# DreamWaterFound/self_commit_ORB-SLAM2

Measured on AMD Instinct MI355X. Metric: frames/s ORB extract+match (1000 feat, 640x480), higher is better.
Workload: dtype u8; 1 GPU; batch of 256 synthetic 640x480 frames per GPU (8 distinct resident batches per step, one launch set per batch), ORB extract (1000 feat, 8 levels, FAST 20/7) + brute-force Hamming SearchByBoW of consecutive frames; batch_per_gpu=256, streams=3, width=640, height=480, nfeatures=1000, parallelism=frames sharded, 1 rank(s), no data-path collective

## Files before the change

### self_commit_orb-slam2_amd/csrc/orbx_extractor.hip

```cpp
#include <math.h>
#include <stdarg.h>
#include <stdio.h>
#include <stdlib.h>
#include <string.h>

#include <algorithm>
#include <atomic>
#include <chrono>
#include <condition_variable>
#include <functional>
#include <memory>
#include <mutex>
#include <thread>
#include <vector>

#include "orbx_internal.h"

static thread_local char g_err[512] = "";

void orbx_set_error(const char *fmt, ...)
{
    va_list ap;
    va_start(ap, fmt);
    vsnprintf(g_err, sizeof(g_err), fmt, ap);
// ... 40 lines not shown
    OrbxGeom geom;
    bool geomValid = false;
    std::vector<uint8_t> binHost;
    std::vector<uint32_t> rsHost;
    std::vector<OrbxFcCell> fcHost;
    OrbxDevBuf<OrbxPyrTile> ptDev;
    int ptBatchW = 0, ptBatchH = 0;
    int ptTiles = 0, ptLds = 0, ptTab = 0;
    int nodeCap = 512;
    hipStream_t stream = nullptr;
    hipEvent_t ev[ORBX_PROF_RING][ST_COUNT + 1] = {};
    bool profiling = false;
    int profCount = 0;
    bool debugTaps = false;
    DevBuf<OrbxGeom> geomDev;
    DevBuf<uint8_t> binDev, pyr, blur, score, staging;
    DevBuf<uint32_t> rsDev;
    DevBuf<OrbxFcCell> fcDev;
    DevBuf<int> cellCount, lvlCnt, lvlBase, status;
    DevBuf<uint8_t> outArena[2];
    int *outCntP[2] = {nullptr, nullptr};
    int *outStP[2] = {nullptr, nullptr};
    orbx_keypoint *outKpP[2] = {nullptr, nullptr};
    uint8_t *outDescP[2] = {nullptr, nullptr};
    size_t arenaKpOff = 0, arenaDescOff = 0, arenaBytes = 0;
    hipEvent_t consumerEv[2] = {nullptr, nullptr};
    hipEvent_t pyrConsumerEv = nullptr;
    int cur = 0;
    DevBuf<uint32_t> cellSlots, ptBuf, labBuf;
    DevBuf<OrbxLevelKp> lvlKp;
    int allocBatch = 0;
    int lastBatch = 0;
    bool lastPyrFast = false;
    bool lastChunked = false;
    const uint8_t *lastImg0 = nullptr;
    int lastStride = 0;
    size_t lastFramePitch = 0;
    uint8_t *hostStaging = nullptr;
    size_t hostStagingBytes = 0;
    int stagingStride = 0;
    size_t stagingFramePitch = 0;
    uint8_t *hostOut = nullptr;
    size_t hostOutBytes = 0;
    hipGraph_t sgGraph[2] = {nullptr, nullptr};
    hipGraphExec_t sgExec[2] = {nullptr, nullptr};
    bool sgValid = false;
    bool sgDisabled = false;
    struct Combiner *comb = nullptr;
    bool combDisabled = false;
    orbx_extractor *expectPartner = nullptr;
    bool isEngine = false;
    size_t hostPyrOff = 0;
    bool hostPyrValid = false;
    bool hostSynced = false;
    bool lastCombined = false;
    struct PipeSlot {
        uint8_t *hostIn = nullptr; size_t hostInBytes = 0;
        DevBuf<uint8_t> devIn;
        uint8_t *hostRes = nullptr; size_t hostResBytes = 0;
        const uint8_t **ptrTab = nullptr; size_t ptrTabBytes = 0;
        hipEvent_t evUp = nullptr, evKern = nullptr, evDown = nullptr;
        int batch = 0, cap = 0;
        size_t offKp = 0, offDesc = 0, offSt = 0;
    } pipe[2];
    int pipeHead = 0, pipeCount = 0;
    double pipeUs[4] = {0, 0, 0, 0};
// ... 195 lines not shown
            if (((ln.w + 3) >> 2) * ((dy - (int)h->rsHost[(size_t)lv.bandOff + b] + 7) >> 3) > ORBX_BAND_MAX_ITEMS) {
                orbx_set_error("level %d (%dx%d): a pyramid band resizes more than %d work items of level %d", l, lv.w, lv.h, ORBX_BAND_MAX_ITEMS, l + 1);
                return ORBX_ERR_ARG;
            }
        }
        h->rsHost.push_back((uint32_t)ln.h);
    }
    h->rsHost.insert(h->rsHost.end(), 16, 0u);
    if (maxWCell > 64 || maxHCell > 63) { orbx_set_error("cell %dx%d larger than the detector supports", maxWCell, maxHCell); return ORBX_ERR_ARG; }
    g.fcPitch = maxWCell <= 32 ? 48 : maxWCell <= 48 ? 64 : 80;
    g.fcScPitch = maxWCell <= 42 ? 48 : 80;
    {
        int maxAw = 1;
        for (int l = 0; l < nl; l++) {
            const OrbxLevel &lv = g.lv[l];
            const int maxBX = lv.w - ORBX_BORDER;
            for (int cj = 0; cj < lv.nCols; cj++) {
                const int iniX = ORBX_BORDER + cj * lv.wCell, maxX = std::min(iniX + lv.wCell + 6, maxBX);
                maxAw = std::max(maxAw, (maxX - 3) - (iniX + 3));
            }
        }
        g.fcScPitch = maxAw + 2 <= 48 ? 48 : 80;
        if (g.fcScPitch == 80) g.fcPitch = 80;
    }
    { const char *pe = getenv("ORBX_FC_PITCH"); if (pe && atoi(pe) == 80 && g.fcPitch == 64) g.fcPitch = 80; }
    {
        const int units = (maxHCell + 6) * ((maxWCell + 6 + 15) / 16), ns = (units + 63) / 64;
        g.fcNS = ns <= 2 ? 2 : ns <= 3 ? 3 : ns <= 4 ? 4 : 6;
    }
    g.fcInBytes = g.fcPitch * (maxHCell + 6);
    g.fcScBytes = g.fcScPitch * (maxHCell + 2);
    g.fcLdsBytes = g.fcInBytes + g.fcScBytes + (int)align_up((size_t)maxWCell * maxHCell * 2, 16);
    g.pyrFast = g.pyrBand && (size_t)ORBX_PF_WAVES * (size_t)g.fcLdsBytes <= 48 * 1024 ? 1 : 0;
    h->fcHost.assign((size_t)cells, OrbxFcCell{});
    for (int l = 0; l < nl; l++) {
        const OrbxLevel &lv = g.lv[l];
        const int maxBX = lv.w - ORBX_BORDER, maxBY = lv.h - ORBX_BORDER;
        for (int ci = 0; ci < lv.nRows; ci++)
            for (int cj = 0; cj < lv.nCols; cj++) {
                const int cell = ci * lv.nCols + cj;
                OrbxFcCell &e = h->fcHost[(size_t)lv.cellBase + cell];
                const int iniX = ORBX_BORDER + cj * lv.wCell, iniY = ORBX_BORDER + ci * lv.hCell;
                const int maxX = std::min(iniX + lv.wCell + 6, maxBX), maxY = std::min(iniY + lv.hCell + 6, maxBY);
                const int x0 = iniX + 3, x1 = maxX - 3, y0 = iniY + 3, y1 = maxY - 3, aw = x1 - x0, ah = y1 - y0;
                const bool valid = !(iniY >= maxBY - 3 || iniX >= maxBX - 6 || aw <= 0 || ah <= 0);
                e.xy = valid ? ((uint32_t)x0 | ((uint32_t)y0 << 16)) : ((uint32_t)ORBX_EDGE | ((uint32_t)ORBX_EDGE << 16));
                const int ew = valid ? aw : 1, eh = valid ? ah : 1, nu = (ew + 6 + 15) / 16;
                e.dim = (uint32_t)ew | ((uint32_t)eh << 8) | ((uint32_t)l << 16) | (valid ? 1u << 24 : 0u);
                e.inv = (uint32_t)((65536 + nu - 1) / nu); e.units = (uint32_t)nu | ((uint32_t)((eh + 6) * nu) << 8);
                e.pitch = lv.pitch; e.off = (uint32_t)lv.off;
                e.slot = (uint32_t)(lv.slotBase + cell * lv.cellCap); e.cap = (uint32_t)lv.cellCap;
            }
    }
    g.pyrBytes = align_up(off + 256, 256);
    if (maxNodes > 2048) { orbx_set_error("per-level feature quota %d exceeds the quadtree node capacity 2048", maxNodes); return ORBX_ERR_ARG; }
    h->nodeCap = maxNodes <= 256 ? 256 : (maxNodes <= 512 ? 512 : (maxNodes <= 1024 ? 1024 : 2048));
    const long long keyLimit = 1ll << (32 - (h->nodeCap == 256 ? 8 : h->nodeCap == 512 ? 9 : h->nodeCap == 1024 ? 10 : 11));
    for (int l = 0; l < nl; l++)
        if ((long long)g.lv[l].nCols * g.lv[l].nRows * g.lv[l].cellCap >= keyLimit) {
            orbx_set_error("level %d (%dx%d) can hold %lld FAST candidates, the quadtree's sort key %lld at %d nodes per level", l, g.lv[l].w, g.lv[l].h,
                           (long long)g.lv[l].nCols * g.lv[l].nRows * g.lv[l].cellCap, keyLimit - 1, h->nodeCap);
            return ORBX_ERR_ARG;
        }
    return ORBX_OK;
}

// ... 82 lines not shown
    int rc = ensure_geometry(h, W, H, batch);
    if (rc != ORBX_OK) return rc;
    OrbxLaunch L;
    h->cur ^= 1;
    const int cb = h->cur;
    fill_launch(h, L, img0Dev, batch, stride, framePitch, cb);
    const bool prof = h->profiling;
    hipEvent_t *ev = h->ev[h->profCount % ORBX_PROF_RING];
    if (h->pyrConsumerEv) { ORBX_HIP_CHECK(hipStreamWaitEvent(h->stream, h->pyrConsumerEv, 0)); h->pyrConsumerEv = nullptr; }
    ORBX_HIP_CHECK(hipMemsetAsync(h->status.p, 0, (size_t)(batch + 1) * sizeof(int), h->stream));
    if (prof) ORBX_HIP_CHECK(hipEventRecord(ev[0], h->stream));
    static const bool batchTiles = getenv("ORBX_BATCH_PYR_TILES") && getenv("ORBX_BATCH_PYR_TILES")[0] == '1';
    bool tiled = false;
    if (batchTiles && h->allocBatch > 1) {
        if (h->ptBatchW != W || h->ptBatchH != H) {
            std::vector<OrbxPyrTile> plan;
            h->ptTiles = 0;
            if (plan_pyramid_tiles(h, plan, h->ptTiles, h->ptLds, h->ptTab)) {
                if ((rc = h->ptDev.ensure(plan.size())) != ORBX_OK) return rc;
                ORBX_HIP_CHECK(hipMemcpy(h->ptDev.p, plan.data(), plan.size() * sizeof(OrbxPyrTile), hipMemcpyHostToDevice));
            } else h->ptTiles = 0;
            h->ptBatchW = W; h->ptBatchH = H;
        }
        if (h->ptTiles > 0) {
            L.pyrTiles = h->ptDev.p; L.pyrTileCount = h->ptTiles; L.pyrTileBuf = h->ptLds; L.pyrTileTab = h->ptTab;
            if ((rc = orbx_launch_pyramid_tiles(L)) != ORBX_OK) return rc;
            tiled = true;
        }
    }
    const char *es = getenv("ORBX_PYR_SPLIT");
    L.pyrBand = !tiled && h->geom.pyrBand && !(es && es[0] == '1');
    const char *ef = getenv("ORBX_FAST_SPLIT");
    const bool pyrFast = L.pyrBand && orbx_pyr_fast_applies(L) && !(ef && ef[0] == '1');
    const int nJoin = pyrFast ? std::min(ORBX_PF_JOIN_LEVELS, h->geom.nlevels) : 0;
    if (L.pyrBand) {
        for (int l = 0; l < h->geom.nlevels; l++)
            if ((rc = l < nJoin ? orbx_launch_pyr_band_fast(L, l) : orbx_launch_pyr_band(L, l)) != ORBX_OK) return rc;
    } else if (!tiled)
        for (int l = 1; l < h->geom.nlevels; l++)
            if ((rc = orbx_launch_resize(L, l)) != ORBX_OK) return rc;
    if (prof) ORBX_HIP_CHECK(hipEventRecord(ev[ST_PYR + 1], h->stream));
    L.fcCellFirst = nJoin < h->geom.nlevels ? h->geom.lv[nJoin].cellBase : h->geom.cellsPerFrame;
    if (L.fcCellFirst < h->geom.cellsPerFrame && (rc = orbx_launch_fast_cells(L)) != ORBX_OK) return rc;
    if (prof) ORBX_HIP_CHECK(hipEventRecord(ev[ST_FAST + 1], h->stream));
    if ((rc = orbx_launch_octree(L)) != ORBX_OK) return rc;
    if (prof) ORBX_HIP_CHECK(hipEventRecord(ev[ST_OCTREE + 1], h->stream));
    if (prof) ORBX_HIP_CHECK(hipEventRecord(ev[ST_ORIENT + 1], h->stream));
    if (!L.pyrBand && (rc = orbx_launch_blur(L)) != ORBX_OK) return rc;
    if (prof) ORBX_HIP_CHECK(hipEventRecord(ev[ST_BLUR + 1], h->stream));
    if (h->consumerEv[cb]) { ORBX_HIP_CHECK(hipStreamWaitEvent(h->stream, h->consumerEv[cb], 0)); h->consumerEv[cb] = nullptr; }
    if ((rc = orbx_launch_orient_describe(L)) != ORBX_OK) return rc;
    if (prof) { ORBX_HIP_CHECK(hipEventRecord(ev[ST_DESC + 1], h->stream)); h->profCount++; }
    h->lastBatch = batch; h->lastImg0 = img0Dev; h->lastStride = stride; h->lastFramePitch = framePitch;
    h->lastCombined = false; h->hostSynced = false; h->lastChunked = false; h->lastPyrFast = pyrFast;
    return ORBX_OK;
}

extern "C" int orbx_debug_last_batch_pyr_fast(orbx_extractor *h) { return h && h->lastPyrFast ? 1 : 0; }

static int host_copy_threads()
{
    static const int n = [] {
        const char *e = getenv("ORBX_HOST_COPY_THREADS");
        int v = e && *e ? atoi(e) : (int)std::min(16u, std::max(1u, std::thread::hardware_concurrency() / 2));
        return v < 1 ? 1 : v > 64 ? 64 : v;
    }();
    return n;
}
struct CopyPool {
    std::mutex m;
    std::mutex jm;
    std::condition_variable cvWork, cvDone;
    std::vector<std::thread> workers;
    std::function<void(int, int)> job;
    int n = 0, parts = 0, gen = 0, pending = 0;
    bool stop = false;
    void worker(int id)
    {
        int seen = 0;
        for (;;) {
            std::function<void(int, int)> fn;
            int n_, parts_;
            {
                std::unique_lock<std::mutex> lk(jm);
                cvWork.wait(lk, [&] { return stop || gen != seen; });
                if (stop) return;
                seen = gen; fn = job; n_ = n; parts_ = parts;
            }
            if (id < parts_) fn((int)((long long)n_ * id / parts_), (int)((long long)n_ * (id + 1) / parts_));
            {
                std::lock_guard<std::mutex> lk(jm);
// ... 1504 lines not shown
```

### self_commit_orb-slam2_amd/csrc/orbx_internal.h

```cpp
#ifndef ORBX_INTERNAL_H
#define ORBX_INTERNAL_H

#include <hip/hip_runtime.h>
#include <cstring>
#include <stdint.h>

#include "../../include/orbx.h"

#define ORBX_MAX_LEVELS 12
#define ORBX_EDGE 19
#define ORBX_BORDER 16
#define ORBX_HALF_PATCH 15
#define ORBX_PATCH 31
#define ORBX_CELL_W 30
#define ORBX_MAX_INI 8

#define ORBX_DEV_ERR_PTCAP 1
#define ORBX_DEV_ERR_NODECAP 2
#define ORBX_DEV_ERR_KPCAP 4

struct OrbxLevel {
    int w, h, pitch;
    int off;
    int nCols, nRows, wCell, hCell;
// ... 10 lines not shown
    int bandOff;
    uint32_t bandDivNc, bandDivG4;
    double rsScaleX, rsScaleY;
    int rsColOff, rsRowOff;
    int patchSize;
    float scale;
};

struct OrbxGeom {
    int nlevels, W, H;
    int iniTh, minTh;
    int cellsPerFrame, slotsPerFrame, kpPerFrame, outCap;
    int blurTiles;
    int fcPitch, fcScPitch, fcNS;
    int fcInBytes, fcScBytes, fcLdsBytes;
    size_t pyrBytes;
    int pyrBand;
    int pyrFast;
    uint32_t taps[7];
    int umax[16];
    OrbxLevel lv[ORBX_MAX_LEVELS];
};

#define ORBX_BAND_MAX_ITEMS (1 << 14)
static inline uint32_t orbx_band_div(int n)
{
    uint32_t S = 14;
    while ((1u << (S - 14)) < (uint32_t)n) S++;
    const uint32_t m = (uint32_t)((((uint64_t)1 << S) + (uint64_t)n - 1) / (uint64_t)n);
    return m | (S << 20);
}

#define ORBX_PF_WAVES 4
#define ORBX_PF_JOIN_LEVELS 2
static inline int orbx_fast_blocks(int cells, int K) { return (cells + ORBX_PF_WAVES * K - 1) / (ORBX_PF_WAVES * K); }
static inline size_t orbx_pyr_fast_lds(const OrbxGeom &g, int l)
{
    const size_t band = (size_t)(g.lv[l].bandH + 6) * (size_t)g.lv[l].bandPitch, fast = (size_t)ORBX_PF_WAVES * (size_t)g.fcLdsBytes;
    return band > fast ? band : fast;
}

struct OrbxFcCell {
    uint32_t xy;
    uint32_t dim;
    int32_t pitch;
    uint32_t off;
    uint32_t slot;
    uint32_t cap;
    uint32_t inv;
    uint32_t units;
};
#define ORBX_FC_CELLS_PER_WAVE 4

struct OrbxPyrTile { short cx0, cy0, cx1, cy1, ox0, oy0, ox1, oy1; };

struct OrbxCombMember {
    const uint8_t *srcImg;
    uint8_t *devImg;
    uint8_t *devPyr;
    uint8_t *devArena;
    uint8_t *hostOut;
    uint8_t *hostPyr;
};

struct OrbxLevelKp { uint16_t x, y; uint8_t score, pad[3]; float angle, ca, sb; };

void orbx_set_error(const char *fmt, ...);
#define ORBX_HIP_CHECK(expr)                                                                           \
    do {                                                                                               \
        hipError_t e_ = (expr);                                                                        \
        if (e_ != hipSuccess) {                                                                        \
            orbx_set_error("%s failed: %s (%s:%d)", #expr, hipGetErrorString(e_), __FILE__, __LINE__); \
            return ORBX_ERR_HIP;                                                                       \
        }                                                                                              \
    } while (0)

struct OrbxLaunch {
    hipStream_t stream;
    const OrbxGeom *geomDev;
    const OrbxGeom *geom;
    int batch;
    const uint8_t *img0;
    int img0Stride;
    size_t img0FramePitch;
    uint8_t *pyr, *blur, *score;
    size_t blurBytes;
    const uint8_t *binTab;
    const uint32_t *rsTab;
    const OrbxFcCell *fcCells;
    int fcCellFirst = 0;
    int *cellCount;
    uint32_t *cellSlots;
    uint32_t *ptBuf, *labBuf;
    OrbxLevelKp *lvlKp;
    int *lvlCnt;
    int *outBase;
    orbx_keypoint *outKp;
    uint8_t *outDesc;
    int *outCnt;
    int *status;
    int *outStatus;
    int nodeCap;
    bool pyrBand = false;
    const OrbxCombMember *combTab = nullptr;
    OrbxCombMember *combTabCopy = nullptr;
    unsigned *combSync = nullptr;
    unsigned long long *combFlag = nullptr;
    size_t combKpOff = 0, combDescOff = 0;
    const OrbxPyrTile *pyrTiles = nullptr; int pyrTileCount = 0, pyrTileBuf = 0, pyrTileTab = 0;
    hipGraph_t graph = nullptr;
    hipGraphNode_t deps[2] = {nullptr, nullptr};
    int ndeps = 0;
    hipGraphNode_t *node = nullptr;
};

int orbx_launch_resize(const OrbxLaunch &L, int level);
int orbx_launch_pyr_band(const OrbxLaunch &L, int level);
bool orbx_pyr_fast_applies(const OrbxLaunch &L);
int orbx_launch_pyr_band_fast(const OrbxLaunch &L, int level);
int orbx_launch_pyramid_tiles(const OrbxLaunch &L);
int orbx_launch_comb_upload(const OrbxLaunch &L, uint8_t *stagingDev);
int orbx_launch_comb_finish(const OrbxLaunch &L);
int orbx_launch_fast_cells(const OrbxLaunch &L);
int orbx_launch_octree(const OrbxLaunch &L);
int orbx_launch_blur(const OrbxLaunch &L);
int orbx_launch_octree_blur(const OrbxLaunch &L, bool *fused);
int orbx_launch_gather_frames(hipStream_t stream, const uint8_t *const *framesPinnedTab, int batch, int W, int H, int srcStride, uint8_t *dst, int dstStride, size_t framePitch, bool aligned16);
int orbx_launch_orient_describe(const OrbxLaunch &L);

hipStream_t orbx_extractor_stream_internal(orbx_extractor *h);
bool orbx_extractor_host_complete_internal(orbx_extractor *h, int *status);
int orbx_extractor_host_count_internal(orbx_extractor *h);
const orbx_keypoint *orbx_extractor_host_keypoints_internal(orbx_extractor *h);
void orbx_extractor_set_consumer_event_internal(orbx_extractor *h, hipEvent_t ev);
const int *orbx_extractor_status_word_internal(orbx_extractor *h);


template <typename T> struct OrbxDevBuf {
    T *p = nullptr;
    size_t n = 0;
    int ensure(size_t count)
    {
        if (count <= n) return ORBX_OK;
        if (p) (void)hipFree(p);
        p = nullptr; n = 0;
        ORBX_HIP_CHECK(hipMalloc((void **)&p, count * sizeof(T)));
        n = count;
        return ORBX_OK;
    }
    void release() { if (p) (void)hipFree(p); p = nullptr; n = 0; }
};

// ... 148 lines not shown
```

### self_commit_orb-slam2_amd/csrc/orbx_kernels.hip

```cpp
#include <algorithm>
#include "orbx_internal.h"

namespace {

struct OdTables {
    float pat[256][4];
    uint32_t disc[64][4];
};
constexpr int8_t kPattern[1024] = {
#include "orb_pattern.inc"
};
constexpr int kUmax[16] = {15, 15, 15, 15, 14, 14, 14, 13, 13, 12, 11, 10, 9, 8, 6, 3};
constexpr OdTables make_od_tables()
{
    OdTables t{};
    for (int i = 0; i < 256; i++) {
        t.pat[i][0] = (float)kPattern[4 * i]; t.pat[i][2] = (float)kPattern[4 * i + 1];
        t.pat[i][1] = (float)kPattern[4 * i + 2]; t.pat[i][3] = (float)kPattern[4 * i + 3];
    }
    for (int ml = 0; ml < 64; ml++)
        for (int j = 0; j < 4; j++) {
            const int mr = ml >> 1, mh = ml & 1;
            uint32_t m = 0u;
            if (mr < 31) {
// ... 478 lines not shown
    }
    if (dbg) {
        const int keepBit = anyIni ? 0x2000 : 0x1000;
        base = 0;
        for (int i0 = 0; i0 < nc; i0 += 64) {
            const int i = i0 + lane;
            bool keep = false;
            int code = 0;
            if (i < nc) { code = cand[i]; keep = (code & keepBit) != 0; }
            const unsigned long long m = __ballot(keep);
            if (keep) {
                const int r = (code >> 6) & 63, c = code & 63;
                const uint32_t v = scT[(r + 1) * SP + c + 4];
                const int idx = base + __popcll(m & ((1ull << lane) - 1ull));
                if (idx < cellCap) slot[idx] = (uint32_t)(x0 + c - ORBX_BORDER) | ((uint32_t)(y0 + r - ORBX_BORDER) << 12) | (v << 24);
            }
            base += __popcll(m);
        }
    }
    if (lane == 0) *cnt = min(base, cellCap);
    fc_wave_sync();
    FC_STAMP(10);
    if (PROF && lane == 0) {
        unsigned long long *rec = prof + 32 + ((size_t)f * cellsPerFrame + ci) * 16;
        for (int i = 0; i < 12; i++) { rec[i] = pacc[i]; pacc[i] = 0; }
        rec[12] = (unsigned long long)pRetry; rec[13] = (unsigned long long)pNc1; rec[14] = (unsigned long long)pNc2; rec[15] = (unsigned long long)min(base, cellCap);
    }
    }
}
#undef FC_STAMP
#undef FC_REQUEST

template <int P, int SP, int NS, bool PROF = false, bool DBG = false>
__global__ __launch_bounds__(64) void k_fast_cells(const OrbxFcCell *__restrict__ cells, int cell0, int K, int cellsPerFrame, int slotsPerFrame, size_t pyrBytes, int iniTh, int minTh,
                                                   int inBytes, int scBytes, const uint8_t *__restrict__ img0, int img0Stride, size_t img0FramePitch,
                                                   const uint8_t *__restrict__ pyr, uint8_t *__restrict__ scoreDbg, int *__restrict__ cellCount,
                                                   uint32_t *__restrict__ cellSlots, unsigned long long *__restrict__ prof)
{
    extern __shared__ __attribute__((aligned(16))) uint8_t lds[];
    unsigned long long tStart = 0;
    if (PROF) tStart = __builtin_amdgcn_s_memtime();
    XCD_REMAP_XY(bx, f);
    const int cFirst = cell0 + bx * K;
    fast_cells_body<P, SP, NS, PROF, DBG>(cells, cFirst, min(cFirst + K, cellsPerFrame), f, lds, (int)threadIdx.x, cellsPerFrame, slotsPerFrame, pyrBytes, iniTh, minTh, inBytes, scBytes,
                                          img0, img0Stride, img0FramePitch, pyr, scoreDbg, cellCount, cellSlots, prof, tStart);
}

struct OtBox { short x0, y0, x1, y1; };

template <typename T> __device__ __forceinline__ T wave_incl_scan(T v, int lane)
{
#pragma unroll
    for (int o = 1; o < 64; o <<= 1) {
        T u = __shfl_up(v, o);
        if (lane >= o) v += u;
    }
    return v;
}

template <int BT = 256, typename T> __device__ T block_exscan(T *arr, int n, T *wsum )
{
    const int tid = threadIdx.x, lane = tid & 63, w = tid >> 6;
    const int per = (n + BT - 1) / BT;
    const int b = tid * per;
    T s = 0;
    for (int k = 0; k < per; k++) if (b + k < n) s += arr[b + k];
    T inc = wave_incl_scan(s, lane);
    if (lane == 63) wsum[w] = inc;
    __syncthreads();
    T off = 0, total = 0;
#pragma unroll
    for (int i = 0; i < BT / 64; i++) { const T v = wsum[i]; off += i < w ? v : (T)0; total += v; }
    T run = off + inc - s;
    for (int k = 0; k < per; k++)
        if (b + k < n) { T v = arr[b + k]; arr[b + k] = run; run += v; }
    __syncthreads();
    return total;
// ... 963 lines not shown
{
    const size_t ldsBytes = 2 * (size_t)L.pyrTileBuf + (size_t)L.pyrTileTab;
    static size_t ldsGranted[64];
    int dev = 0;
    (void)hipGetDevice(&dev);
    size_t &granted = ldsGranted[dev & 63];
    if (ldsBytes > std::max<size_t>(granted, 48 * 1024)) {
        const hipError_t e = hipFuncSetAttribute((const void *)k_pyramid_tiles, hipFuncAttributeMaxDynamicSharedMemorySize, (int)ldsBytes);
        if (e != hipSuccess) { orbx_set_error("hipFuncSetAttribute(k_pyramid_tiles) failed: %s", hipGetErrorString(e)); return ORBX_ERR_HIP; }
        granted = ldsBytes;
    }
    return emit(L, k_pyramid_tiles, dim3((unsigned)L.pyrTileCount, (unsigned)L.batch), dim3(256), ldsBytes, L.geomDev, L.img0, L.img0Stride, L.img0FramePitch, L.pyr, L.rsTab,
                L.pyrTiles, L.pyrTileBuf, L.status);
}

int orbx_launch_comb_upload(const OrbxLaunch &L, uint8_t *stagingDev)
{
    const size_t units = L.img0FramePitch >> 4;
    const unsigned blocks = (unsigned)std::min<size_t>(std::max<size_t>((units + 255) / 256, 1), 256);
    return emit(L, k_comb_upload, dim3(blocks, (unsigned)L.batch), dim3(256), 0, L.combTab, L.combTabCopy, stagingDev, L.img0FramePitch);
}

int orbx_launch_comb_finish(const OrbxLaunch &L)
{
    const size_t units = (L.geom->pyrBytes + L.img0FramePitch) >> 4;
    const unsigned blocks = (unsigned)std::min<size_t>(std::max<size_t>((units + 2047) / 2048, 1), 64);
    return emit(L, k_comb_finish, dim3(blocks, (unsigned)L.batch), dim3(256), 0, (const OrbxCombMember *)L.combTabCopy, L.outCnt, L.outStatus, L.outKp, L.outDesc, L.geom->outCap, L.pyr, L.geom->pyrBytes, L.img0,
                L.img0FramePitch, L.combKpOff, L.combDescOff, 0, L.combSync, L.combFlag);
}

static unsigned long long *g_fcProf = nullptr;
extern "C" void orbx_debug_fast_cells_profile(unsigned long long *dev32) { g_fcProf = dev32; }

static int fc_cells_per_wave(int batch)
{
    static const int kEnv = getenv("ORBX_FC_CELLS_PER_WAVE") ? atoi(getenv("ORBX_FC_CELLS_PER_WAVE")) : 0;
    return kEnv > 0 ? kEnv : (batch >= 32 ? ORBX_FC_CELLS_PER_WAVE : 1);
}

int orbx_launch_fast_cells(const OrbxLaunch &L)
{
    const OrbxGeom &g = *L.geom;
    const int K = fc_cells_per_wave(L.batch);
    dim3 grid((unsigned)((g.cellsPerFrame - L.fcCellFirst + K - 1) / K), (unsigned)L.batch);
    const size_t ldsBytes = (size_t)g.fcLdsBytes;
#define FC_ARGS L.fcCells, L.fcCellFirst, K, g.cellsPerFrame, g.slotsPerFrame, g.pyrBytes, g.iniTh, g.minTh, g.fcInBytes, g.fcScBytes, L.img0, L.img0Stride, L.img0FramePitch, L.pyr, L.score, L.cellCount, L.cellSlots
#define FC_LAUNCH(PP, SS, NN) do { if (L.score) return emit(L, k_fast_cells<PP, SS, NN, false, true>, grid, dim3(64), ldsBytes, FC_ARGS, (unsigned long long *)nullptr); \
    if (g_fcProf) return emit(L, k_fast_cells<PP, SS, NN, true, false>, grid, dim3(64), ldsBytes, FC_ARGS, g_fcProf); \
    return emit(L, k_fast_cells<PP, SS, NN, false, false>, grid, dim3(64), ldsBytes, FC_ARGS, (unsigned long long *)nullptr); } while (0)
#define FC_LAUNCH_P(PP, SS) switch (g.fcNS) { case 2: FC_LAUNCH(PP, SS, 2); case 3: FC_LAUNCH(PP, SS, 3); case 4: FC_LAUNCH(PP, SS, 4); default: FC_LAUNCH(PP, SS, 6); }
    if (g.fcPitch == 48 && g.fcScPitch == 48) FC_LAUNCH_P(48, 48)
    if (g.fcPitch == 64 && g.fcScPitch == 48) FC_LAUNCH_P(64, 48)
    if (g.fcPitch == 80 && g.fcScPitch == 48) FC_LAUNCH_P(80, 48)
    if (g.fcPitch != 80 || g.fcScPitch != 80) { orbx_set_error("detector LDS pitches %d / %d have no kernel instantiation", g.fcPitch, g.fcScPitch); return ORBX_ERR_STATE; }
    FC_LAUNCH_P(80, 80)
#undef FC_LAUNCH_P
#undef FC_LAUNCH
#undef FC_ARGS
}

int orbx_launch_octree(const OrbxLaunch &L)
{
    dim3 grid((unsigned)(L.geom->nlevels + (L.combTab ? ORBX_OCTREE_COPY_BLOCKS : 0)), (unsigned)L.batch);
#define OT_LAUNCH(NC) return emit(L, k_octree<NC>, grid, dim3(256), 0, L.geomDev, L.cellCount, L.cellSlots, L.binTab, L.ptBuf, L.labBuf, L.lvlKp, L.lvlCnt, L.status, L.combTab, \
                                  (const uint8_t *)L.pyr, L.pyrBand ? L.outBase : (int *)nullptr)
    if (L.nodeCap <= 256) OT_LAUNCH(256);
    if (L.nodeCap <= 512) OT_LAUNCH(512);
    if (L.nodeCap <= 1024) OT_LAUNCH(1024);
    OT_LAUNCH(2048);
#undef OT_LAUNCH
}

int orbx_launch_octree_blur(const OrbxLaunch &L, bool *fused)
{
    *fused = false;
    if (!L.combTab || L.nodeCap > 512) return ORBX_OK;
    unsigned tapSum = 0;
    for (int i = 0; i < 7; i++) tapSum += L.geom->taps[i];
    const int tpb = OB_THREADS / 64;
// ... 15 lines not shown
    *fused = true;
#define OB_LAUNCH(NC, CL) return emit(L, k_octree_blur<NC, CL>, grid, dim3(OB_THREADS), lds, L.geomDev, L.cellCount, L.cellSlots, L.binTab, L.ptBuf, L.labBuf, L.lvlKp, L.lvlCnt, L.status, L.combTab, \
                                      L.img0, L.img0Stride, L.img0FramePitch, L.pyr, L.blur)
    if (L.nodeCap <= 256) { if (tapSum > 256u) OB_LAUNCH(256, true); OB_LAUNCH(256, false); }
    if (tapSum > 256u) OB_LAUNCH(512, true);
    OB_LAUNCH(512, false);
#undef OB_LAUNCH
}

int orbx_launch_blur(const OrbxLaunch &L)
{
    dim3 grid((unsigned)L.geom->blurTiles, (unsigned)L.batch);
    unsigned tapSum = 0;
    for (int i = 0; i < 7; i++) tapSum += L.geom->taps[i];
    if (tapSum > 256u) return emit(L, k_blur<true>, grid, dim3(64), 0, L.geomDev, L.img0, L.img0Stride, L.img0FramePitch, L.pyr, L.blur, L.lvlCnt, L.outBase);
    return emit(L, k_blur<false>, grid, dim3(64), 0, L.geomDev, L.img0, L.img0Stride, L.img0FramePitch, L.pyr, L.blur, L.lvlCnt, L.outBase);
}

int orbx_launch_pyr_band(const OrbxLaunch &L, int l)
{
    const OrbxGeom &g = *L.geom;
    const OrbxLevel &lv = g.lv[l];
    const dim3 grid((unsigned)((lv.h + lv.bandH - 1) / lv.bandH), (unsigned)L.batch);
    const size_t lds = (size_t)(lv.bandH + 6) * lv.bandPitch;
    const int readable = l > 0 ? lv.pitch : (L.img0FramePitch >= (size_t)L.img0Stride * (size_t)lv.h ? L.img0Stride : lv.w);
    unsigned tapSum = 0;
    for (int i = 0; i < 7; i++) tapSum += g.taps[i];
    if (tapSum > 256u) return emit(L, k_pyr_band<true>, grid, dim3(PB_THREADS), lds, L.geomDev, l, L.img0, L.img0Stride, L.img0FramePitch, readable, L.pyr, L.blur, L.rsTab, L.outBase);
    return emit(L, k_pyr_band<false>, grid, dim3(PB_THREADS), lds, L.geomDev, l, L.img0, L.img0Stride, L.img0FramePitch, readable, L.pyr, L.blur, L.rsTab, L.outBase);
}

bool orbx_pyr_fast_applies(const OrbxLaunch &L) { return L.geom->pyrBand && L.geom->pyrFast && !L.score && !g_fcProf; }

int orbx_launch_pyr_band_fast(const OrbxLaunch &L, int l)
{
    const OrbxGeom &g = *L.geom;
    const OrbxLevel &lv = g.lv[l];
    const int K = fc_cells_per_wave(L.batch), ncell = lv.nCols * lv.nRows;
    const int nBands = (lv.h + lv.bandH - 1) / lv.bandH;
    const dim3 grid((unsigned)(nBands + orbx_fast_blocks(ncell, K)), (unsigned)L.batch);
    const size_t lds = orbx_pyr_fast_lds(g, l);
    const int readable = l > 0 ? lv.pitch : (L.img0FramePitch >= (size_t)L.img0Stride * (size_t)lv.h ? L.img0Stride : lv.w);
    unsigned tapSum = 0;
    for (int i = 0; i < 7; i++) tapSum += g.taps[i];
#define PF_ARGS L.geomDev, l, L.img0, L.img0Stride, L.img0FramePitch, readable, L.pyr, L.blur, L.rsTab, L.outBase, nBands, L.fcCells, K, lv.cellBase, lv.cellBase + ncell, g.cellsPerFrame, \
                g.slotsPerFrame, g.pyrBytes, g.iniTh, g.minTh, g.fcInBytes, g.fcScBytes, g.fcLdsBytes, L.cellCount, L.cellSlots
#define PF_LAUNCH(PP, SS, NN) do { if (tapSum > 256u) return emit(L, k_pyr_band_fast<true, PP, SS, NN>, grid, dim3(PB_THREADS), lds, PF_ARGS); \
    return emit(L, k_pyr_band_fast<false, PP, SS, NN>, grid, dim3(PB_THREADS), lds, PF_ARGS); } while (0)
#define PF_LAUNCH_P(PP, SS) switch (g.fcNS) { case 2: PF_LAUNCH(PP, SS, 2); case 3: PF_LAUNCH(PP, SS, 3); case 4: PF_LAUNCH(PP, SS, 4); default: PF_LAUNCH(PP, SS, 6); }
    if (g.fcPitch == 48 && g.fcScPitch == 48) PF_LAUNCH_P(48, 48)
    if (g.fcPitch == 64 && g.fcScPitch == 48) PF_LAUNCH_P(64, 48)
    if (g.fcPitch == 80 && g.fcScPitch == 48) PF_LAUNCH_P(80, 48)
    if (g.fcPitch != 80 || g.fcScPitch != 80) { orbx_set_error("detector LDS pitches %d / %d have no kernel instantiation", g.fcPitch, g.fcScPitch); return ORBX_ERR_STATE; }
    PF_LAUNCH_P(80, 80)
#undef PF_LAUNCH_P
#undef PF_LAUNCH
#undef PF_ARGS
}

int orbx_launch_orient_describe(const OrbxLaunch &L)
{
    dim3 grid((unsigned)((L.geom->kpPerFrame + OD_WPB - 1) / OD_WPB), (unsigned)L.batch);
    const OrbxGeom &g = *L.geom;
    OdLevels A;
    memset(&A, 0, sizeof(A));
    A.nlevels = g.nlevels; A.kpPerFrame = g.kpPerFrame; A.outCap = g.outCap; A.pyrBytes = g.pyrBytes;
    for (int l = 0; l < ORBX_MAX_LEVELS; l++) A.kpBase[l] = 0x7fffffff;
    for (int l = 0; l < g.nlevels; l++) { A.kpBase[l] = g.lv[l].kpBase; A.off[l] = g.lv[l].off; A.pitch[l] = g.lv[l].pitch; A.patch[l] = g.lv[l].patchSize; A.scale[l] = g.lv[l].scale; }
    for (int i = 0; i < 16; i++)
        if (g.umax[i] != kUmax[i]) { orbx_set_error("disc half-widths differ from the compiled table"); return ORBX_ERR_STATE; }
    return emit(L, k_orient_describe, grid, dim3(64 * OD_WPB), 0, A, L.img0, L.img0Stride, L.img0FramePitch, L.pyr, L.blur, L.lvlKp, L.lvlCnt, L.combTab ? (const int *)nullptr : (const int *)L.outBase, L.outKp, L.outDesc,
                L.outCnt, L.status, L.outStatus);
}
```

Before: 316,800 frames/s.

## Plan per-level FAST join and cells-per-wave from occupancy instead of fixed constants

```diff
diff --git a/self_commit_orb-slam2_amd/csrc/orbx_extractor.hip b/self_commit_orb-slam2_amd/csrc/orbx_extractor.hip
--- a/self_commit_orb-slam2_amd/csrc/orbx_extractor.hip
+++ b/self_commit_orb-slam2_amd/csrc/orbx_extractor.hip
@@ -96,6 +96,8 @@
     int allocBatch = 0;
     int lastBatch = 0;
     bool lastPyrFast = false;
+    OrbxPfPlan lastPfPlan = {};
+    int pfWaveSlots[ORBX_MAX_LEVELS + 1] = {};
     bool lastChunked = false;
     const uint8_t *lastImg0 = nullptr;
     int lastStride = 0;
@@ -357,6 +359,7 @@
     g.fcScBytes = g.fcScPitch * (maxHCell + 2);
     g.fcLdsBytes = g.fcInBytes + g.fcScBytes + (int)align_up((size_t)maxWCell * maxHCell * 2, 16);
     g.pyrFast = g.pyrBand && (size_t)ORBX_PF_WAVES * (size_t)g.fcLdsBytes <= 48 * 1024 ? 1 : 0;
+    memset(h->pfWaveSlots, 0, sizeof(h->pfWaveSlots));
     h->fcHost.assign((size_t)cells, OrbxFcCell{});
     for (int l = 0; l < nl; l++) {
         const OrbxLevel &lv = g.lv[l];
@@ -505,16 +508,19 @@
     L.pyrBand = !tiled && h->geom.pyrBand && !(es && es[0] == '1');
     const char *ef = getenv("ORBX_FAST_SPLIT");
     const bool pyrFast = L.pyrBand && orbx_pyr_fast_applies(L) && !(ef && ef[0] == '1');
-    const int nJoin = pyrFast ? std::min(ORBX_PF_JOIN_LEVELS, h->geom.nlevels) : 0;
+    OrbxPfPlan pf = {};
+    if (pyrFast) {
+        if ((rc = orbx_pyr_fast_plan(h->geom, batch, h->pfWaveSlots, &pf)) != ORBX_OK) return rc;
+        L.pfPlan = &pf;
+    }
     if (L.pyrBand) {
         for (int l = 0; l < h->geom.nlevels; l++)
-            if ((rc = l < nJoin ? orbx_launch_pyr_band_fast(L, l) : orbx_launch_pyr_band(L, l)) != ORBX_OK) return rc;
+            if ((rc = (pf.joinMask >> l & 1u) ? orbx_launch_pyr_band_fast(L, l) : orbx_launch_pyr_band(L, l)) != ORBX_OK) return rc;
     } else if (!tiled)
         for (int l = 1; l < h->geom.nlevels; l++)
             if ((rc = orbx_launch_resize(L, l)) != ORBX_OK) return rc;
     if (prof) ORBX_HIP_CHECK(hipEventRecord(ev[ST_PYR + 1], h->stream));
-    L.fcCellFirst = nJoin < h->geom.nlevels ? h->geom.lv[nJoin].cellBase : h->geom.cellsPerFrame;
-    if (L.fcCellFirst < h->geom.cellsPerFrame && (rc = orbx_launch_fast_cells(L)) != ORBX_OK) return rc;
+    if ((rc = orbx_launch_fast_cells(L)) != ORBX_OK) return rc;
     if (prof) ORBX_HIP_CHECK(hipEventRecord(ev[ST_FAST + 1], h->stream));
     if ((rc = orbx_launch_octree(L)) != ORBX_OK) return rc;
     if (prof) ORBX_HIP_CHECK(hipEventRecord(ev[ST_OCTREE + 1], h->stream));
@@ -525,11 +531,18 @@
     if ((rc = orbx_launch_orient_describe(L)) != ORBX_OK) return rc;
     if (prof) { ORBX_HIP_CHECK(hipEventRecord(ev[ST_DESC + 1], h->stream)); h->profCount++; }
     h->lastBatch = batch; h->lastImg0 = img0Dev; h->lastStride = stride; h->lastFramePitch = framePitch;
-    h->lastCombined = false; h->hostSynced = false; h->lastChunked = false; h->lastPyrFast = pyrFast;
+    h->lastCombined = false; h->hostSynced = false; h->lastChunked = false; h->lastPyrFast = pf.joinMask != 0; h->lastPfPlan = pf;
     return ORBX_OK;
 }
 
 extern "C" int orbx_debug_last_batch_pyr_fast(orbx_extractor *h) { return h && h->lastPyrFast ? 1 : 0; }
+extern "C" unsigned orbx_debug_last_batch_pyr_fast_plan(orbx_extractor *h, int *cellsPerWave, int *waveSlots, int *ownSlots)
+{
+    if (!h) return 0u;
+    if (ownSlots) *ownSlots = h->lastPfPlan.ownSlots;
+    for (int l = 0; l < ORBX_MAX_LEVELS; l++) { if (cellsPerWave) cellsPerWave[l] = h->lastPfPlan.K[l]; if (waveSlots) waveSlots[l] = h->lastPfPlan.waveSlots[l]; }
+    return h->lastPfPlan.joinMask;
+}
 
 static int host_copy_threads()
 {
diff --git a/self_commit_orb-slam2_amd/csrc/orbx_internal.h b/self_commit_orb-slam2_amd/csrc/orbx_internal.h
--- a/self_commit_orb-slam2_amd/csrc/orbx_internal.h
+++ b/self_commit_orb-slam2_amd/csrc/orbx_internal.h
@@ -66,7 +66,32 @@
 }
 
 #define ORBX_PF_WAVES 4
+#define ORBX_PF_ROUNDS_X4 8
+#define ORBX_PF_JOIN_ROUNDS_X4 7
+#define ORBX_PF_SMALL_SET_ROUNDS_X4 16
 #define ORBX_PF_JOIN_LEVELS 2
+struct OrbxPfPlan {
+    int K[ORBX_MAX_LEVELS];
+    unsigned joinMask;
+    int waveSlots[ORBX_MAX_LEVELS];
+    int ownSlots;
+};
+static inline int orbx_pf_cells_per_wave(int cells, int batch, int waveSlots, int roundsX4)
+{
+    if (batch < 32) return 1;
+    for (int K = 4; K > 1; K >>= 1)
+        if (4ll * cells * batch >= (long long)roundsX4 * waveSlots * K) return K;
+    return 1;
+}
+static inline bool orbx_pf_joined(int level, int cells, int cellsPerFrame, int batch, int jointSlots, int ownSlots, int joinRoundsX4)
+{
+    if ((long long)cellsPerFrame * batch < (long long)ORBX_PF_SMALL_SET_ROUNDS_X4 * ownSlots) return level < ORBX_PF_JOIN_LEVELS;
+    return jointSlots >= ownSlots && (long long)cells * batch >= (long long)joinRoundsX4 * ownSlots;
+}
+struct OrbxFcSections {
+    int n;
+    int blockEnd[ORBX_MAX_LEVELS], cell0[ORBX_MAX_LEVELS], cellEnd[ORBX_MAX_LEVELS], K[ORBX_MAX_LEVELS];
+};
 static inline int orbx_fast_blocks(int cells, int K) { return (cells + ORBX_PF_WAVES * K - 1) / (ORBX_PF_WAVES * K); }
 static inline size_t orbx_pyr_fast_lds(const OrbxGeom &g, int l)
 {
@@ -122,7 +147,7 @@
     const uint8_t *binTab;
     const uint32_t *rsTab;
     const OrbxFcCell *fcCells;
-    int fcCellFirst = 0;
+    const OrbxPfPlan *pfPlan = nullptr;
     int *cellCount;
     uint32_t *cellSlots;
     uint32_t *ptBuf, *labBuf;
@@ -152,6 +177,7 @@
 int orbx_launch_pyr_band(const OrbxLaunch &L, int level);
 bool orbx_pyr_fast_applies(const OrbxLaunch &L);
 int orbx_launch_pyr_band_fast(const OrbxLaunch &L, int level);
+int orbx_pyr_fast_plan(const OrbxGeom &g, int batch, int *waveSlots, OrbxPfPlan *plan);
 int orbx_launch_pyramid_tiles(const OrbxLaunch &L);
 int orbx_launch_comb_upload(const OrbxLaunch &L, uint8_t *stagingDev);
 int orbx_launch_comb_finish(const OrbxLaunch &L);
diff --git a/self_commit_orb-slam2_amd/csrc/orbx_kernels.hip b/self_commit_orb-slam2_amd/csrc/orbx_kernels.hip
--- a/self_commit_orb-slam2_amd/csrc/orbx_kernels.hip
+++ b/self_commit_orb-slam2_amd/csrc/orbx_kernels.hip
@@ -534,7 +534,7 @@
 #undef FC_REQUEST
 
 template <int P, int SP, int NS, bool PROF = false, bool DBG = false>
-__global__ __launch_bounds__(64) void k_fast_cells(const OrbxFcCell *__restrict__ cells, int cell0, int K, int cellsPerFrame, int slotsPerFrame, size_t pyrBytes, int iniTh, int minTh,
+__global__ __launch_bounds__(64) void k_fast_cells(const OrbxFcCell *__restrict__ cells, const OrbxFcSections S, int cellsPerFrame, int slotsPerFrame, size_t pyrBytes, int iniTh, int minTh,
                                                    int inBytes, int scBytes, const uint8_t *__restrict__ img0, int img0Stride, size_t img0FramePitch,
                                                    const uint8_t *__restrict__ pyr, uint8_t *__restrict__ scoreDbg, int *__restrict__ cellCount,
                                                    uint32_t *__restrict__ cellSlots, unsigned long long *__restrict__ prof)
@@ -543,8 +543,14 @@
     unsigned long long tStart = 0;
     if (PROF) tStart = __builtin_amdgcn_s_memtime();
     XCD_REMAP_XY(bx, f);
-    const int cFirst = cell0 + bx * K;
-    fast_cells_body<P, SP, NS, PROF, DBG>(cells, cFirst, min(cFirst + K, cellsPerFrame), f, lds, (int)threadIdx.x, cellsPerFrame, slotsPerFrame, pyrBytes, iniTh, minTh, inBytes, scBytes,
+    int K = S.K[0], c0 = S.cell0[0], cEnd = S.cellEnd[0], b0 = 0;
+    if (S.n > 1 && bx >= S.blockEnd[0]) {
+        int s = 1;
+        while (s + 1 < S.n && bx >= S.blockEnd[s]) s++;
+        K = S.K[s]; c0 = S.cell0[s]; cEnd = S.cellEnd[s]; b0 = S.blockEnd[s - 1];
+    }
+    const int cFirst = c0 + (bx - b0) * K;
+    fast_cells_body<P, SP, NS, PROF, DBG>(cells, cFirst, min(cFirst + K, cEnd), f, lds, (int)threadIdx.x, cellsPerFrame, slotsPerFrame, pyrBytes, iniTh, minTh, inBytes, scBytes,
                                           img0, img0Stride, img0FramePitch, pyr, scoreDbg, cellCount, cellSlots, prof, tStart);
 }
 
@@ -1574,19 +1580,38 @@
 static unsigned long long *g_fcProf = nullptr;
 extern "C" void orbx_debug_fast_cells_profile(unsigned long long *dev32) { g_fcProf = dev32; }
 
+static int fc_cells_per_wave_knob()
+{
+    static const int kEnv = getenv("ORBX_FC_CELLS_PER_WAVE") ? atoi(getenv("ORBX_FC_CELLS_PER_WAVE")) : 0;
+    return kEnv;
+}
 static int fc_cells_per_wave(int batch)
 {
-    static const int kEnv = getenv("ORBX_FC_CELLS_PER_WAVE") ? atoi(getenv("ORBX_FC_CELLS_PER_WAVE")) : 0;
+    const int kEnv = fc_cells_per_wave_knob();
     return kEnv > 0 ? kEnv : (batch >= 32 ? ORBX_FC_CELLS_PER_WAVE : 1);
 }
 
 int orbx_launch_fast_cells(const OrbxLaunch &L)
 {
     const OrbxGeom &g = *L.geom;
-    const int K = fc_cells_per_wave(L.batch);
-    dim3 grid((unsigned)((g.cellsPerFrame - L.fcCellFirst + K - 1) / K), (unsigned)L.batch);
+    OrbxFcSections S;
+    memset(&S, 0, sizeof(S));
+    if (!L.pfPlan) {
+        const int K = fc_cells_per_wave(L.batch);
+        S.n = 1; S.cell0[0] = 0; S.cellEnd[0] = g.cellsPerFrame; S.K[0] = K; S.blockEnd[0] = (g.cellsPerFrame + K - 1) / K;
+    } else {
+        for (int l = 0; l < g.nlevels; l++) {
+            if (L.pfPlan->joinMask >> l & 1u) continue;
+            const int K = L.pfPlan->K[l], c0 = g.lv[l].cellBase, c1 = c0 + g.lv[l].nCols * g.lv[l].nRows;
+            if (S.n > 0 && S.cellEnd[S.n - 1] == c0 && S.K[S.n - 1] == K) S.cellEnd[S.n - 1] = c1;
+            else { S.cell0[S.n] = c0; S.cellEnd[S.n] = c1; S.K[S.n] = K; S.n++; }
+        }
+        for (int i = 0, b = 0; i < S.n; i++) S.blockEnd[i] = b += (S.cellEnd[i] - S.cell0[i] + S.K[i] - 1) / S.K[i];
+        if (S.n == 0) return ORBX_OK;
+    }
+    dim3 grid((unsigned)S.blockEnd[S.n - 1], (unsigned)L.batch);
     const size_t ldsBytes = (size_t)g.fcLdsBytes;
-#define FC_ARGS L.fcCells, L.fcCellFirst, K, g.cellsPerFrame, g.slotsPerFrame, g.pyrBytes, g.iniTh, g.minTh, g.fcInBytes, g.fcScBytes, L.img0, L.img0Stride, L.img0FramePitch, L.pyr, L.score, L.cellCount, L.cellSlots
+#define FC_ARGS L.fcCells, S, g.cellsPerFrame, g.slotsPerFrame, g.pyrBytes, g.iniTh, g.minTh, g.fcInBytes, g.fcScBytes, L.img0, L.img0Stride, L.img0FramePitch, L.pyr, L.score, L.cellCount, L.cellSlots
 #define FC_LAUNCH(PP, SS, NN) do { if (L.score) return emit(L, k_fast_cells<PP, SS, NN, false, true>, grid, dim3(64), ldsBytes, FC_ARGS, (unsigned long long *)nullptr); \
     if (g_fcProf) return emit(L, k_fast_cells<PP, SS, NN, true, false>, grid, dim3(64), ldsBytes, FC_ARGS, g_fcProf); \
     return emit(L, k_fast_cells<PP, SS, NN, false, false>, grid, dim3(64), ldsBytes, FC_ARGS, (unsigned long long *)nullptr); } while (0)
@@ -1668,30 +1693,112 @@
 
 bool orbx_pyr_fast_applies(const OrbxLaunch &L) { return L.geom->pyrBand && L.geom->pyrFast && !L.score && !g_fcProf; }
 
+typedef void (*PfKernel)(const OrbxGeom *, int, const uint8_t *, int, size_t, int, uint8_t *, uint8_t *, const uint32_t *, int *, int, const OrbxFcCell *, int, int, int, int, int, size_t, int, int,
+                         int, int, int, int *, uint32_t *);
+static PfKernel pf_kernel(const OrbxGeom &g)
+{
+    unsigned tapSum = 0;
+    for (int i = 0; i < 7; i++) tapSum += g.taps[i];
+    const bool clamp = tapSum > 256u;
+#define PF_PICK(PP, SS, NN) return clamp ? (PfKernel)k_pyr_band_fast<true, PP, SS, NN> : (PfKernel)k_pyr_band_fast<false, PP, SS, NN>
+#define PF_PICK_P(PP, SS) switch (g.fcNS) { case 2: PF_PICK(PP, SS, 2); case 3: PF_PICK(PP, SS, 3); case 4: PF_PICK(PP, SS, 4); default: PF_PICK(PP, SS, 6); }
+    if (g.fcPitch == 48 && g.fcScPitch == 48) PF_PICK_P(48, 48)
+    if (g.fcPitch == 64 && g.fcScPitch == 48) PF_PICK_P(64, 48)
+    if (g.fcPitch == 80 && g.fcScPitch == 48) PF_PICK_P(80, 48)
+    if (g.fcPitch != 80 || g.fcScPitch != 80) { orbx_set_error("detector LDS pitches %d / %d have no kernel instantiation", g.fcPitch, g.fcScPitch); return nullptr; }
+    PF_PICK_P(80, 80)
+#undef PF_PICK_P
+#undef PF_PICK
+}
+
 int orbx_launch_pyr_band_fast(const OrbxLaunch &L, int l)
 {
     const OrbxGeom &g = *L.geom;
     const OrbxLevel &lv = g.lv[l];
-    const int K = fc_cells_per_wave(L.batch), ncell = lv.nCols * lv.nRows;
+    const int K = L.pfPlan ? L.pfPlan->K[l] : fc_cells_per_wave(L.batch), ncell = lv.nCols * lv.nRows;
     const int nBands = (lv.h + lv.bandH - 1) / lv.bandH;
     const dim3 grid((unsigned)(nBands + orbx_fast_blocks(ncell, K)), (unsigned)L.batch);
     const size_t lds = orbx_pyr_fast_lds(g, l);
     const int readable = l > 0 ? lv.pitch : (L.img0FramePitch >= (size_t)L.img0Stride * (size_t)lv.h ? L.img0Stride : lv.w);
-    unsigned tapSum = 0;
-    for (int i = 0; i < 7; i++) tapSum += g.taps[i];
-#define PF_ARGS L.geomDev, l, L.img0, L.img0Stride, L.img0FramePitch, readable, L.pyr, L.blur, L.rsTab, L.outBase, nBands, L.fcCells, K, lv.cellBase, lv.cellBase + ncell, g.cellsPerFrame, \
-                g.slotsPerFrame, g.pyrBytes, g.iniTh, g.minTh, g.fcInBytes, g.fcScBytes, g.fcLdsBytes, L.cellCount, L.cellSlots
-#define PF_LAUNCH(PP, SS, NN) do { if (tapSum > 256u) return emit(L, k_pyr_band_fast<true, PP, SS, NN>, grid, dim3(PB_THREADS), lds, PF_ARGS); \
-    return emit(L, k_pyr_band_fast<false, PP, SS, NN>, grid, dim3(PB_THREADS), lds, PF_ARGS); } while (0)
-#define PF_LAUNCH_P(PP, SS) switch (g.fcNS) { case 2: PF_LAUNCH(PP, SS, 2); case 3: PF_LAUNCH(PP, SS, 3); case 4: PF_LAUNCH(PP, SS, 4); default: PF_LAUNCH(PP, SS, 6); }
-    if (g.fcPitch == 48 && g.fcScPitch == 48) PF_LAUNCH_P(48, 48)
-    if (g.fcPitch == 64 && g.fcScPitch == 48) PF_LAUNCH_P(64, 48)
-    if (g.fcPitch == 80 && g.fcScPitch == 48) PF_LAUNCH_P(80, 48)
-    if (g.fcPitch != 80 || g.fcScPitch != 80) { orbx_set_error("detector LDS pitches %d / %d have no kernel instantiation", g.fcPitch, g.fcScPitch); return ORBX_ERR_STATE; }
-    PF_LAUNCH_P(80, 80)
-#undef PF_LAUNCH_P
-#undef PF_LAUNCH
-#undef PF_ARGS
+    const PfKernel kern = pf_kernel(g);
+    if (!kern) return ORBX_ERR_STATE;
+    return emit(L, kern, grid, dim3(PB_THREADS), lds, L.geomDev, l, L.img0, L.img0Stride, L.img0FramePitch, readable, L.pyr, L.blur, L.rsTab, L.outBase, nBands, L.fcCells, K, lv.cellBase,
+                lv.cellBase + ncell, g.cellsPerFrame, g.slotsPerFrame, g.pyrBytes, g.iniTh, g.minTh, g.fcInBytes, g.fcScBytes, g.fcLdsBytes, L.cellCount, L.cellSlots);
+}
+
+static int pyr_fast_wave_slots(const OrbxGeom &g, int l, int *slots)
+{
+    const PfKernel kern = pf_kernel(g);
+    if (!kern) return ORBX_ERR_STATE;
+    int dev = 0, cus = 0, blocks = 0;
+    ORBX_HIP_CHECK(hipGetDevice(&dev));
+    ORBX_HIP_CHECK(hipDeviceGetAttribute(&cus, hipDeviceAttributeMultiprocessorCount, dev));
+    ORBX_HIP_CHECK(hipOccupancyMaxActiveBlocksPerMultiprocessor(&blocks, (const void *)kern, PB_THREADS, orbx_pyr_fast_lds(g, l)));
+    *slots = std::max(1, cus * blocks * ORBX_PF_WAVES);
+    return ORBX_OK;
+}
+
+static int fast_cells_wave_slots(const OrbxGeom &g, int *slots)
+{
+    const void *kern = nullptr;
+#define FC_PICK(PP, SS) switch (g.fcNS) { case 2: kern = (const void *)k_fast_cells<PP, SS, 2, false, false>; break; case 3: kern = (const void *)k_fast_cells<PP, SS, 3, false, false>; break; \
+                                          case 4: kern = (const void *)k_fast_cells<PP, SS, 4, false, false>; break; default: kern = (const void *)k_fast_cells<PP, SS, 6, false, false>; }
+    if (g.fcPitch == 48 && g.fcScPitch == 48) FC_PICK(48, 48)
+    else if (g.fcPitch == 64 && g.fcScPitch == 48) FC_PICK(64, 48)
+    else if (g.fcPitch == 80 && g.fcScPitch == 48) FC_PICK(80, 48)
+    else if (g.fcPitch == 80 && g.fcScPitch == 80) FC_PICK(80, 80)
+    else { orbx_set_error("detector LDS pitches %d / %d have no kernel instantiation", g.fcPitch, g.fcScPitch); return ORBX_ERR_STATE; }
+#undef FC_PICK
+    int dev = 0, cus = 0, blocks = 0;
+    ORBX_HIP_CHECK(hipGetDevice(&dev));
+    ORBX_HIP_CHECK(hipDeviceGetAttribute(&cus, hipDeviceAttributeMultiprocessorCount, dev));
+    ORBX_HIP_CHECK(hipOccupancyMaxActiveBlocksPerMultiprocessor(&blocks, kern, 64, (size_t)g.fcLdsBytes));
+    *slots = std::max(1, cus * blocks);
+    return ORBX_OK;
+}
+
+static void pf_env_list(const char *name, int *K, int n)
+{
+    const char *e = getenv(name);
+    for (int l = 0; e && *e && l < n; l++) {
+        char *end = nullptr;
+        const long v = strtol(e, &end, 10);
+        if (end == e) break;
+        if (v >= 1 && v <= 64) K[l] = (int)v;
+        e = *end == ',' ? end + 1 : end;
+    }
+}
+static int pf_env_rounds_x4(const char *name, int dflt)
+{
+    const char *e = getenv(name);
+    return e && *e ? (int)(atof(e) * 4.0 + 0.5) : dflt;
+}
+
+int orbx_pyr_fast_plan(const OrbxGeom &g, int batch, int *waveSlots, OrbxPfPlan *plan)
+{
+    memset(plan, 0, sizeof(*plan));
+    const int roundsX4 = pf_env_rounds_x4("ORBX_PF_ROUNDS", ORBX_PF_ROUNDS_X4), joinX4 = pf_env_rounds_x4("ORBX_PF_JOIN_ROUNDS", ORBX_PF_JOIN_ROUNDS_X4);
+    const int kKnob = fc_cells_per_wave_knob();
+    int rc;
+    if (!waveSlots[g.nlevels] && (rc = fast_cells_wave_slots(g, &waveSlots[g.nlevels])) != ORBX_OK) return rc;
+    const int ownSlots = plan->ownSlots = waveSlots[g.nlevels];
+    for (int l = 0; l < g.nlevels; l++) {
+        if (!waveSlots[l] && (rc = pyr_fast_wave_slots(g, l, &waveSlots[l])) != ORBX_OK) return rc;
+        plan->waveSlots[l] = waveSlots[l];
+        if (orbx_pf_joined(l, g.lv[l].nCols * g.lv[l].nRows, g.cellsPerFrame, batch, waveSlots[l], ownSlots, joinX4)) plan->joinMask |= 1u << l;
+    }
+    const char *em = getenv("ORBX_PF_JOIN_MASK");
+    if (em && *em) plan->joinMask = (unsigned)strtoul(em, nullptr, 0);
+    plan->joinMask &= (1u << g.nlevels) - 1u;
+    int ownCells = 0;
+    for (int l = 0; l < g.nlevels; l++)
+        if (!(plan->joinMask >> l & 1u)) ownCells += g.lv[l].nCols * g.lv[l].nRows;
+    for (int l = 0; l < g.nlevels; l++) {
+        const bool joined = plan->joinMask >> l & 1u;
+        plan->K[l] = kKnob > 0 ? kKnob : orbx_pf_cells_per_wave(joined ? g.lv[l].nCols * g.lv[l].nRows : ownCells, batch, joined ? waveSlots[l] : ownSlots, roundsX4);
+    }
+    pf_env_list("ORBX_PF_CELLS_PER_WAVE", plan->K, g.nlevels);
+    return ORBX_OK;
 }
 
 int orbx_launch_orient_describe(const OrbxLaunch &L)
```

Result: no change. 317,900 frames/s (median of 4 runs) (+0.3%).
